# google/supersonic

Hardware: AMD Instinct MI355X
Metric: rows/sec filter->project->aggregate, 100M x 8 INT64/DOUBLE (higher is better)
Workload: dtype int64/f64; 1 GPU; Q-FPA-wide: SUM(a+b),COUNT(*),SUM(c),MIN(d),MAX(d0),SUM(d1),SUM(d2*d3) WHERE a>499 over a device-resident 100000000-row x 8-col block per GPU; rows_per_gpu=100000000, parallelism=single GPU, tile_rows=512, grid=768, lds_bytes=35568, specialized_stages=1

## Files before the change

supersonic_amd/csrc/launch.h:

```cpp
#ifndef SSGPU_LAUNCH_H_
#define SSGPU_LAUNCH_H_

#ifndef __HIPCC_RTC__
#include <hip/hip_runtime_api.h>
#include <stdint.h>
#endif
#include "vm.h"

enum SlotKind {
  SLOT_SUM_INT = 0, SLOT_SUM_DD = 1, SLOT_MIN_U64 = 2, SLOT_MAX_U64 = 3, SLOT_MIN_F64 = 4,
  SLOT_MAX_F64 = 5, SLOT_FIRST = 6, SLOT_LAST = 7, SLOT_COUNT = 8
};
enum EmitKind {
  EMIT_U64 = 0, EMIT_I64KEY = 1, EMIT_U32 = 2, EMIT_I32KEY = 3, EMIT_F64 = 4, EMIT_F32 = 5,
  EMIT_DD_F64 = 6, EMIT_DD_F32 = 7, EMIT_U8 = 8,
  EMIT_DDRES_F64 = 9,
  EMIT_CNT_U64 = 20, EMIT_CNT_U32 = 21,
  EMIT_FKEY_F64 = 100, EMIT_FKEY_F32 = 101
};
#define SSGPU_STATE_ARRAYS 8

struct EmitDesc { void* data; uint8_t* is_null; int slot; int out_kind; };

struct GroupKeyOut { void* data; uint8_t* is_null; uint32_t shift, bits, nullbit, width; };
// ... 165 lines not shown
                                    bool prefetch = false);
hipError_t ssgpu_launch_group_resident_rtc(void* handle, const PartAggParams& A, const PlainScatterParams& S, int grid, hipStream_t stream);
hipError_t ssgpu_launch_part_agg_rtc(void* handle, const PartAggParams& P, hipStream_t stream);
void* ssgpu_rtc_specialize_pscat(int device, const PlainScatterParams& S, const PscatGeom& g, std::string* why);
hipError_t ssgpu_launch_part_scatter_plain_rtc(void* handle, const PlainScatterParams& P, const PscatGeom& g, int grid, hipStream_t stream);
void* ssgpu_rtc_function(void* handle);
void ssgpu_rtc_release(void* handle);
void ssgpu_rtc_cached_only(bool on);
void ssgpu_rtc_mode(int mode);
int ssgpu_rtc_current_mode();
bool ssgpu_rtc_pending();
void ssgpu_rtc_trim(int keep);
void ssgpu_rtc_stats(long long* modules, long long* code_bytes, long long* compilations, long long* disk_hits);
#endif
hipError_t ssgpu_pipeline_set_max_lds(int bytes);
hipError_t ssgpu_launch_finish_slots(const VmAccRec* partials, int n_slots, int n_parts, const int* slot_kind,
                                     VmAccRec* out, uint64_t* state , hipStream_t stream,
                                     const EmitDesc* descs = nullptr, int n_out = 0 );
hipError_t ssgpu_launch_slots_to_state(const VmAccRec* recs, int n_slots, const int* slot_kind, uint64_t* state,
                                       hipStream_t stream);
hipError_t ssgpu_launch_fold_state(const uint64_t* images, int n_images, uint64_t* state, int n_slots, const int* slot_kind, hipStream_t stream);
hipError_t ssgpu_launch_fold_emit(const uint64_t* images, int n_images, uint64_t* state, int n_slots, const int* slot_kind, VmAccRec* recs,
                                  const EmitDesc* descs, int n_out, hipStream_t stream);
hipError_t ssgpu_launch_state_to_slots(const uint64_t* state, int n_slots, const int* slot_kind, VmAccRec* recs,
                                       hipStream_t stream);
hipError_t ssgpu_launch_emit_scalar(const VmAccRec* recs, const EmitDesc* descs, int n_out, hipStream_t stream);
hipError_t ssgpu_launch_scan_counts(const uint32_t* in, uint32_t* out, int n, uint64_t* total, hipStream_t stream);
hipError_t ssgpu_launch_group_count(const GroupExtractParams& P, uint32_t* tile_counts, hipStream_t stream);
hipError_t ssgpu_launch_group_extract_lb(const GroupExtractParams& P, unsigned long long* status, uint64_t epoch, unsigned int* ctrl, unsigned int* error_flag, hipStream_t stream);
hipError_t ssgpu_launch_group_extract(const GroupExtractParams& P, hipStream_t stream);
hipError_t ssgpu_launch_fill_u64(uint64_t* p, uint64_t v, size_t n, hipStream_t stream);
hipError_t ssgpu_launch_fill_pattern_u64(uint64_t* p, const uint64_t* pattern, uint32_t plen, size_t n,
                                         hipStream_t stream);
// ... 93 lines not shown
```

supersonic_amd/csrc/pipeline_kernels.hip:

```cpp
#ifndef __HIPCC_RTC__
#include <hip/hip_runtime.h>
#include <stdint.h>
#endif
#include "vm.h"
#include "launch.h"
#ifdef SSGPU_RTC_NINSTR
#include "rtc_prog.h"
#endif

typedef unsigned long long u64;
typedef long long i64;
typedef unsigned int u32;
typedef int i32;
typedef unsigned char u8;

#ifdef SSGPU_PC_PROFILE
#define PC_PROF(...) __VA_ARGS__
#else
#define PC_PROF(...)
#endif
struct LdsBase {
  __device__ __forceinline__ char* operator+(u32 off) const {
    return (char*)(__attribute__((address_space(3))) char*)off;
  }
// ... 753 lines not shown
      a = dd_add_d(a, u2d(state[3 * n_slots + s]));
      r.v0 = d2u(a.hi); r.v1 = d2u(a.lo);
    } break;
    case SLOT_MIN_U64: r.v0 = state[4 * n_slots + s] ^ 0x8000000000000000ull; break;
    case SLOT_MAX_U64: r.v0 = state[5 * n_slots + s] ^ 0x8000000000000000ull; break;
    case SLOT_MIN_F64: r.v0 = state[6 * n_slots + s]; break;
    case SLOT_MAX_F64: r.v0 = state[7 * n_slots + s]; break;
    case SLOT_FIRST: r.v0 = state[s]; r.v1 = state[4 * n_slots + s] ^ 0x8000000000000000ull; break;
    case SLOT_LAST: r.v0 = state[s]; r.v1 = state[5 * n_slots + s] ^ 0x8000000000000000ull; break;
    default: break;
  }
  return r;
}

__device__ __forceinline__ void emit_scalar_one(const EmitDesc d, const VmAccRec r);
__global__ __launch_bounds__(256) void ssgpu_finish_slots_kernel(const VmAccRec* __restrict__ partials, int n_slots,
                                                                 int n_parts, const int* __restrict__ slot_kind,
                                                                 VmAccRec* __restrict__ out, u64* __restrict__ state,
                                                                 const EmitDesc* __restrict__ descs, int n_out) {
  __shared__ VmAccRec tree[256];
  const int s = blockIdx.x, t = threadIdx.x;
  const int kind = slot_kind[s];
  VmAccRec acc; acc.v0 = 0; acc.v1 = 0; acc.cnt = 0; acc.pad = 0;
  if (kind == SLOT_SUM_DD) { acc.v0 = d2u(-0.0); acc.v1 = d2u(0.0); }
  for (int i = t; i < n_parts; i += 256) {
    const VmAccRec r = partials[((size_t)(i / VM_WAVES) * n_slots + s) * VM_WAVES + (i % VM_WAVES)];
    combine_rec(kind, acc, r);
  }
  tree[t] = acc;
  __syncthreads();
  for (int stride = 128; stride > 0; stride >>= 1) {
    if (t < stride) { VmAccRec a = tree[t]; combine_rec(kind, a, tree[t + stride]); tree[t] = a; }
    __syncthreads();
  }
  if (t == 0) { out[s] = tree[0]; if (state) slot_to_state(tree[0], kind, s, n_slots, state); }
  if (descs)
    for (int i = t; i < n_out; i += 256) { const EmitDesc d = descs[i]; if (d.slot == s) emit_scalar_one(d, tree[0]); }
}

__global__ void ssgpu_slots_to_state_kernel(const VmAccRec* __restrict__ recs, int n_slots,
                                            const int* __restrict__ slot_kind, u64* __restrict__ state) {
  int s = blockIdx.x * blockDim.x + threadIdx.x;
  if (s >= n_slots) return;
  slot_to_state(recs[s], slot_kind[s], s, n_slots, state);
}
__global__ void ssgpu_state_to_slots_kernel(const u64* __restrict__ state, int n_slots,
                                            const int* __restrict__ slot_kind, VmAccRec* __restrict__ recs) {
  int s = blockIdx.x * blockDim.x + threadIdx.x;
  if (s >= n_slots) return;
  recs[s] = state_to_slot(state, slot_kind[s], s, n_slots);
}

// ... 955 lines not shown
  e = hipFuncSetAttribute(reinterpret_cast<const void*>(ssgpu_part_agg_kernel<SSGPU_PART_MAX_WORDS>), hipFuncAttributeMaxDynamicSharedMemorySize, bytes);
  if (e != hipSuccess) return e;
  return hipFuncSetAttribute(reinterpret_cast<const void*>(ssgpu_part_agg_kernel<16>), hipFuncAttributeMaxDynamicSharedMemorySize, bytes);
}
hipError_t ssgpu_pipeline_set_max_lds(int bytes) {
  hipError_t e;
  e = hipFuncSetAttribute(reinterpret_cast<const void*>(ssgpu_pipeline_kernel<1, false>), hipFuncAttributeMaxDynamicSharedMemorySize, bytes); if (e != hipSuccess) return e;
  e = hipFuncSetAttribute(reinterpret_cast<const void*>(ssgpu_pipeline_kernel<2, false>), hipFuncAttributeMaxDynamicSharedMemorySize, bytes); if (e != hipSuccess) return e;
  e = hipFuncSetAttribute(reinterpret_cast<const void*>(ssgpu_pipeline_kernel<4, false>), hipFuncAttributeMaxDynamicSharedMemorySize, bytes); if (e != hipSuccess) return e;
  e = hipFuncSetAttribute(reinterpret_cast<const void*>(ssgpu_pipeline_kernel<1, true>), hipFuncAttributeMaxDynamicSharedMemorySize, bytes); if (e != hipSuccess) return e;
  e = hipFuncSetAttribute(reinterpret_cast<const void*>(ssgpu_pipeline_kernel<2, true>), hipFuncAttributeMaxDynamicSharedMemorySize, bytes); if (e != hipSuccess) return e;
  e = hipFuncSetAttribute(reinterpret_cast<const void*>(ssgpu_pipeline_kernel<4, true>), hipFuncAttributeMaxDynamicSharedMemorySize, bytes);
  return e;
}
hipError_t ssgpu_launch_finish_slots(const VmAccRec* partials, int n_slots, int n_parts, const int* slot_kind,
                                     VmAccRec* out, uint64_t* state, hipStream_t stream, const EmitDesc* descs, int n_out) {
  hipLaunchKernelGGL(ssgpu_finish_slots_kernel, dim3(n_slots), dim3(256), 0, stream, partials, n_slots, n_parts, slot_kind, out, (u64*)state, descs, n_out);
  return hipGetLastError();
}
hipError_t ssgpu_launch_slots_to_state(const VmAccRec* recs, int n_slots, const int* slot_kind, uint64_t* state, hipStream_t stream) {
  int blocks = (n_slots + 63) / 64;
  hipLaunchKernelGGL(ssgpu_slots_to_state_kernel, dim3(blocks), dim3(64), 0, stream, recs, n_slots, slot_kind, (u64*)state);
  return hipGetLastError();
}
__device__ __forceinline__ void fold_state_slot(const u64* __restrict__ images, int n_images, u64* __restrict__ state, int n_slots, int kind, int s);
__global__ __launch_bounds__(64) void ssgpu_fold_state_kernel(const u64* __restrict__ images, int n_images, u64* __restrict__ state,
                                                              int n_slots, const int* __restrict__ slot_kind) {
  const int s = blockIdx.x * 64 + threadIdx.x;
  if (s >= n_slots) return;
  fold_state_slot(images, n_images, state, n_slots, slot_kind[s], s);
}
__device__ __forceinline__ void fold_state_slot(const u64* __restrict__ images, int n_images, u64* __restrict__ state, int n_slots, int kind, int s) {
// ... 132 lines not shown
```

supersonic_amd/csrc/runtime.cpp:

```cpp
#include <hip/hip_runtime_api.h>

#include <atomic>
#include <chrono>
#include <map>
#include <tuple>
#include <set>
#include <mutex>
#include <stdio.h>
#include <string.h>
#include <algorithm>
#include <cmath>
#include <string>
#include <unistd.h>
#include <thread>
#include <unordered_set>
#include <vector>
#include <deque>
#include <functional>

#include "engine.h"

using namespace ssgpu;

#define HIP_TRY(ctx, expr)                                                          \
// ... 27 lines not shown
  int64_t part_wgs_per_cu = 0;
  int64_t part_lds_target = 0;
  int64_t sort_records = 1;
  int64_t sort_hybrid = 1;
  int64_t group_slab = 1;
  int64_t group_scout = 1;
  int64_t group_scout_rows = 8 << 20;
  int64_t group_resident = 1;
  int64_t group_dense = 1;
  int64_t dense_parts = 0;
  int64_t dense_min_rows = 1 << 16;
  int64_t async_handoff = 1;
  int64_t lazy_feedback = 0;
  int64_t part_prefetch = 1;
  int64_t fuse_emit = 1;
  int64_t pscat_pipe = 1;
  int64_t pscat_threads = 0, pscat_rows = 0, pscat_wgs = 0;
  int64_t part_plain = 1;
  int64_t sort_compact = 1;
  int64_t sort_hi_digits = 4;
  int64_t part_agg_lds = 0;
  int64_t profile = 1;
  int64_t profile_total = 1;
  int64_t debug_timing = 0;
  int64_t specialize = 3;
  int64_t specialize_min_rows = 1 << 22;
};

struct MemQuota { int64_t limit = -1; int64_t used = 0; };
static thread_local MemQuota* g_quota = nullptr;
// ... 79 lines not shown
      (void)hipGetLastError();
      int dev = -1;
      if (hipGetDevice(&dev) == hipSuccess && g_pool.trim(dev) > 0) e = hipMalloc(&p, want);
    }
    if (e == hipSuccess) { cap = want; q = Q; g_dev_bytes.fetch_add((long long)want); if (q) q->used += (int64_t)want; } else p = nullptr;
    return e;
  }
  template <typename T> T* as() const { return reinterpret_cast<T*>(p); }
};

struct PinnedBuf {
  void* p = nullptr;
  size_t cap = 0;
  ~PinnedBuf() { drop(); }
  void drop() { if (p) { (void)hipHostFree(p); g_pinned_bytes.fetch_sub((long long)cap); } p = nullptr; cap = 0; }
  hipError_t ensure(size_t bytes) {
    if (bytes <= cap && p) return hipSuccess;
    drop();
    size_t want = std::max<size_t>(bytes, 256);
    hipError_t e = hipHostMalloc(&p, want, hipHostMallocDefault);
    if (e == hipSuccess) { cap = want; g_pinned_bytes.fetch_add((long long)want); } else p = nullptr;
    return e;
  }
};

struct OutCol { DevBuf data, nulls; bool nullable = false; uint32_t width = 8; };

struct StageExec {
  DevBuf prog_main, prog_count;
  struct RtcSlot {
    void* h = nullptr; bool tried = false; uint32_t static_lds = 0, tag = 0;
    int missed_mode = -1;
    bool stronger_mode_now() const { if (h || missed_mode < 0) return false; const int m = ssgpu_rtc_current_mode(); return missed_mode == 1 && m != 1; }
    bool pending = false; std::chrono::steady_clock::time_point next_poll{};
    void drop() { if (h) ssgpu_rtc_release(h); h = nullptr; tried = false; static_lds = 0; tag = 0; pending = false; missed_mode = -1; }
// ... 48 lines not shown
    uint32_t span[8] = {0}, stride[8] = {0};
    uint64_t slots = 0;
    uint32_t np = 0, cap = 0;
    uint64_t chunk_bytes = 0;
    int64_t widened = 0;
  } dense;
  DevBuf dense_dom, dense_flags;
  void* dense_table = nullptr;
  std::vector<DevBuf> rowid_tmp;
  std::vector<DevBuf> jkeys, jkeys_hi, jrows, jmisc;
  std::vector<DevBuf> jcounts, jstarts, jslot_of_row, jrows_sorted;
  DevBuf jx_offsets, jx_lhs_idx, jx_rhs_row;
  std::vector<VmJoin> vm_joins;
  uint32_t capacity = 0;
  DevBuf error_flag;
  DevBuf debug, debug_pc, total2;
  DevBuf skeys_a, skeys_b, skeys_c, sidx_a, sidx_b, shist, soffs, seg_id, sstatus, sticket, srecs, dflag;
  DevBuf rank_first, rank_of_seg, rank_row, rank_own;
  DevBuf seg_counts, seg_offsets, seg_total;
  DevBuf route_scratch;
  uint64_t sort_epoch = 0;
  bool emit_ready = false;
  bool emitted_with_finish = false;
  bool pattern_ready = false;
  DevBuf out_arena;
  std::vector<OutCol> out;
  int64_t out_rows = -1;
  const void* out_rows_dev = nullptr;
  int64_t out_capacity = 0;
  int last_group_shape = 0;
// ... 74 lines not shown
        if (consumed[b]) (void)hipEventDestroy(consumed[b]);
        uploaded[b] = consumed[b] = nullptr; in_flight[b] = false;
      }
    }
  } host_stream;
  struct StreamJob {
    int kind = 0;
    ssgpu_plan* head = nullptr; ssgpu_plan* tail = nullptr;
    std::vector<DevBuf> acc_data, acc_nulls;
    int64_t acc_rows = 0, acc_cap = 0;
    int64_t rows_hint = 0;
  };
  StreamJob* stream_job = nullptr;
  ssgpu_plan* skip_plan = nullptr;
  int64_t run_row_end = 0;
  bool keep_error_flags = false;
  ssgpu_result result;
};

struct ssgpu_block {
  ssgpu_ctx* ctx = nullptr;
  Schema schema;
  int64_t capacity = 0, rows = 0;
  DevBuf arena;
  std::vector<DevBuf> data, nulls;
  ssgpu_dict* dict = nullptr;
};
static const size_t kBlockColumnSkew = 512, kBlockArenaMin = 32u << 20;

static int fail(ssgpu_ctx* ctx, const Status& s) { if (ctx) ctx->err = s.msg; return s.code; }
// ... 82 lines not shown
  else if (k == "part_lds_target") c->part_lds_target = value;
  else if (k == "part_agg_lds") c->part_agg_lds = value;
  else if (k == "group_slab") c->group_slab = value;
  else if (k == "group_resident") c->group_resident = value;
  else if (k == "group_dense") c->group_dense = value;
  else if (k == "dense_parts") c->dense_parts = value;
  else if (k == "dense_min_rows") c->dense_min_rows = value;
  else if (k == "group_scout") c->group_scout = value;
  else if (k == "group_scout_rows") c->group_scout_rows = value;
  else if (k == "part_plain") c->part_plain = value;
  else if (k == "pscat_threads") c->pscat_threads = value;
  else if (k == "pscat_rows") c->pscat_rows = value;
  else if (k == "pscat_wgs") c->pscat_wgs = value;
  else if (k == "pscat_pipe") c->pscat_pipe = value;
  else if (k == "fuse_emit") c->fuse_emit = value;
  else if (k == "part_prefetch") c->part_prefetch = value;
  else if (k == "lazy_feedback") c->lazy_feedback = value;
  else if (k == "async_handoff") c->async_handoff = value;
  else if (k == "sort_records") c->sort_records = value;
  else if (k == "sort_hybrid") c->sort_hybrid = value;
  else if (k == "sort_hi_digits") c->sort_hi_digits = value;
  else if (k == "sort_compact") c->sort_compact = value;
  else if (k == "group_capacity") {
    int64_t cap = 1; while (cap < value) cap <<= 1;
    c->group_capacity = cap;
  } else if (k == "profile") c->profile = value;
  else if (k == "profile_total") c->profile_total = value;
  else if (k == "debug_timing") c->debug_timing = value;
  else if (k == "specialize") c->specialize = value;
  else if (k == "specialize_min_rows") c->specialize_min_rows = value < 0 ? 0 : value;
// ... 453 lines not shown
}

void ssgpu_plan_destroy(ssgpu_plan* p) {
  if (!p) return;
  if (p->skip_plan) { ssgpu_plan* q = p->skip_plan; p->skip_plan = nullptr; ssgpu_plan_destroy(q); }
  if (p->stream_job) {
    ssgpu_plan::StreamJob* j = p->stream_job; p->stream_job = nullptr;
    if (p->ctx && p->ctx->device >= 0) (void)hipStreamSynchronize(p->ctx->stream);
    if (j->tail) ssgpu_plan_destroy(j->tail);
    if (j->head && j->head != p) ssgpu_plan_destroy(j->head);
    delete j;
  }
  if (p->ctx && p->ctx->device >= 0) {
    (void)hipStreamSynchronize(p->ctx->stream);
    if (p->host_stream.open) { (void)hipStreamSynchronize(p->ctx->copy_stream); p->host_stream.drop_events(); p->host_stream.open = false; }
    if (p->ev_begin) { (void)hipEventDestroy(p->ev_begin); g_events.fetch_sub(1); }
    if (p->ev_end) { (void)hipEventDestroy(p->ev_end); g_events.fetch_sub(1); }
    for (int i = 0; i < ssgpu_plan::kEventRing; ++i) {
      if (p->ring0[i]) { (void)hipEventDestroy(p->ring0[i]); g_events.fetch_sub(1); }
      if (p->ring1[i]) { (void)hipEventDestroy(p->ring1[i]); g_events.fetch_sub(1); }
    }
  }
  for (auto& ex : p->exec) { ex.rtc_main.drop(); ex.rtc_pscatter.drop(); ex.rtc_plain.drop(); ex.rtc_part.drop(); ex.rtc_resident.drop(); ex.rtc_hot.drop(); }
  for (auto& ex : p->exec) if (ex.fb_event) { (void)hipEventDestroy(ex.fb_event); ex.fb_event = nullptr; g_events.fetch_sub(1); }
  ssgpu_ctx* c = p->ctx;
  g_live_plans.fetch_sub(1);
  if (c && c->device >= 0) (void)hipSetDevice(c->device);
  tls_park_released = c && c->device >= 0;
  delete p;
  tls_park_released = false;
// ... 91 lines not shown
  ProgramLayout L = layout_program(st.main, c->opt);
  if (ex.prog_main.p && L.K == ex.lay.K) return SSGPU_OK;
  ex.lay = L;
  int rc = upload_program(c, st.main, L, &ex.prog_main, &ex.n_instr_main, &p->host_prog_scratch);
  if (rc != SSGPU_OK) return rc;
  ex.host_prog_main = p->host_prog_scratch;
  if (ex.rtc_main.h) (void)hipStreamSynchronize(c->stream);
  ex.rtc_main.drop(); ex.rtc_why.clear();
  if (!st.count_pass.empty()) {
    LowerOptions o = c->opt; o.tile_rows = VM_TILE_UNIT * 4;
    ex.lay_count = layout_program(st.count_pass, o);
    if (ex.lay_count.K < L.K) { o.tile_rows = VM_TILE_UNIT * L.K; ex.lay_count = layout_program(st.count_pass, o); }
    rc = upload_program(c, st.count_pass, ex.lay_count, &ex.prog_count, &ex.n_instr_count, &p->host_prog_scratch);
    if (rc != SSGPU_OK) return rc;
  }
  HIP_TRY(c, ex.error_flag.ensure(sizeof(uint32_t)));
  return SSGPU_OK;
}

int sort_rows_by_u32(ssgpu_plan* p, StageExec& ex, const uint32_t* keys32, uint64_t n, uint32_t** sorted) {
  ssgpu_ctx* c = p->ctx;
  const uint32_t nt = ssgpu_sort_tiles(n);
  HIP_TRY(c, ex.skeys_a.ensure(std::max<uint64_t>(n, 1) * 8)); HIP_TRY(c, ex.skeys_b.ensure(std::max<uint64_t>(n, 1) * 8));
  HIP_TRY(c, ex.sidx_a.ensure(std::max<uint64_t>(n, 1) * 4)); HIP_TRY(c, ex.sidx_b.ensure(std::max<uint64_t>(n, 1) * 4));
  HIP_TRY(c, ex.shist.ensure((size_t)std::max<uint32_t>(nt, 1) * 256 * 4)); HIP_TRY(c, ex.soffs.ensure((size_t)std::max<uint32_t>(nt, 1) * 256 * 4));
  HIP_TRY(c, ex.total.ensure(8)); HIP_TRY(c, ex.total2.ensure(16));
  uint64_t* ka = ex.skeys_a.as<uint64_t>(); uint64_t* kb = ex.skeys_b.as<uint64_t>();
  uint32_t* ia = ex.sidx_a.as<uint32_t>(); uint32_t* ib = ex.sidx_b.as<uint32_t>();
  HIP_TRY(c, ssgpu_launch_sort_iota(ia, n, c->stream));
  if (n > 0) {
    const unsigned long long init[2] = {0ull, ~0ull};
// ... 363 lines not shown
  }
  P.wg_partials = ex.wg_partials.as<VmAccRec>();
  P.error_flag = ex.error_flag.as<unsigned int>();
  if (c->debug_timing) {
    HIP_TRY(c, ex.debug.ensure((size_t)grid * 4 * 8));
    P.debug = ex.debug.as<unsigned long long>();
  }
  { int rc = attach_pc_profile(c, ex, &P); if (rc != SSGPU_OK) return rc; }
  if (c->profile) HIP_TRY(c, hipEventRecord(p->ev_dom0, c->stream));
  HIP_TRY(c, launch_main(p, st, ex, P, ex.lay.K, grid));
  if (c->profile) HIP_TRY(c, hipEventRecord(p->ev_dom1, c->stream));
  { int rc = print_pc_profile(c, ex, st.main, P.n_instr); if (rc != SSGPU_OK) return rc; }
  int n_emit = 0;
  ex.emitted_with_finish = false;
  if (!stop_at_partial && c->fuse_emit) { const int rc = prepare_scalar_emit(p, si, &n_emit); if (rc != SSGPU_OK) return rc; ex.emitted_with_finish = true; }
  HIP_TRY(c, ssgpu_launch_finish_slots(ex.wg_partials.as<VmAccRec>(), ns, grid * VM_WAVES, ex.slot_kind.as<int>(),
                                       ex.slot_recs.as<VmAccRec>(), stop_at_partial ? ex.state.as<uint64_t>() : nullptr, c->stream,
                                       ex.emitted_with_finish ? ex.emit_descs.as<EmitDesc>() : nullptr, n_emit));
  p->counters.n_launches += 2;
  p->counters.tile_rows = P.tile_rows; p->counters.grid = grid; p->counters.lds_bytes = (int32_t)ex.lay.lds_bytes;
  if (c->debug_timing) {
    std::vector<unsigned long long> dbg((size_t)grid * 4);
    HIP_TRY(c, hipMemcpy(dbg.data(), ex.debug.p, dbg.size() * 8, hipMemcpyDeviceToHost));
    double tot = 0, wait = 0, tiles = 0;
    for (int g = 0; g < grid; ++g) { tot += (double)dbg[g * 4]; wait += (double)dbg[g * 4 + 1]; tiles += (double)dbg[g * 4 + 2]; }
    fprintf(stderr, "[ssgpu debug] grid=%d tiles/wg=%.1f cycles/wg=%.0f wait=%.1f%% cycles/tile=%.0f (wait %.0f)\n", grid, tiles / grid,
            tot / grid, 100.0 * wait / tot, tot / tiles, wait / tiles);
  }
  return SSGPU_OK;
}

static const int64_t kSeqSumPiece = 1 << 21;
static int run_seq_sums(ssgpu_plan* p, Stage& st, StageExec& ex, const InCols& in, const uint32_t* seg_id) {
// ... 1312 lines not shown
static const void* rows_word(const StageExec& ex) { return ex.out_rows_dev ? ex.out_rows_dev : ex.total.p; }
int stage_rows(ssgpu_plan* p, size_t si, int64_t* rows) {
  ssgpu_ctx* c = p->ctx; StageExec& ex = p->exec[si];
  if (ex.out_rows < 0) {
    uint64_t total = 0;
    HIP_TRY(c, hipMemcpyAsync(&total, rows_word(ex), 8, hipMemcpyDeviceToHost, c->stream));
    HIP_TRY(c, hipStreamSynchronize(c->stream));
    ex.out_rows = (int64_t)total;
  }
  *rows = ex.out_rows;
  return SSGPU_OK;
}

int check_error_flags(ssgpu_plan* p);

int check_error_flags(ssgpu_plan* p) {
  ssgpu_ctx* c = p->ctx;
  std::vector<uint32_t> flags(p->exec.size(), 0);
  for (size_t i = 0; i < p->exec.size(); ++i)
    if (p->exec[i].error_flag.p)
      HIP_TRY(c, hipMemcpyAsync(&flags[i], p->exec[i].error_flag.p, 4, hipMemcpyDeviceToHost, c->stream));
  HIP_TRY(c, hipStreamSynchronize(c->stream));
  for (uint32_t& f : flags) {
    if (f & SSGPU_FLAG_NAN_IN_MINMAX) p->nan_seen = true;
    f &= 0xFFu;
  }
  for (uint32_t f : flags) {
    if (f == 3) { c->err = "decoupled look-back: a tile waited for an earlier tile's row count for too long and gave up"; return SSGPU_ERROR_HIP; }
    if (f) {
      c->err = f == 2 ? "Evaluation error: invalid argument of a signaling math expression (negative input of SQRT)"
                      : "Evaluation error: division by zero in a signaling expression";
      return SSGPU_ERROR_EVALUATION_ERROR;
    }
  }
  return SSGPU_OK;
}

// ... 39 lines not shown
  p->exec.clear();
  p->stages = stages; p->describe = describe;
  p->exec.resize(p->stages.size());
  std::vector<ssgpu_column> cols = p->last_cols;
  int rc = run_plan(p, cols.data(), (int32_t)cols.size(), p->last_rows, p->last_base, false);
  if (rc != SSGPU_OK) return rc;
  rc = settle_plan(p);
  if (rc != SSGPU_OK) return rc;
  rc = check_error_flags(p);
  p->nan_seen = false;
  return rc;
}

int run_plan(ssgpu_plan* p, const ssgpu_column* cols, int32_t n_cols, int64_t rows, int64_t row_id_base, bool partial) {
  ssgpu_ctx* c = p->ctx;
  if (!c || c->device < 0) { if (c) c->err = "no gfx950 device bound to this context (bind-only context)"; return SSGPU_ERROR_NO_DEVICE; }
  ssgpu_rtc_mode(!p->cached_only ? 0 : p->background && rows >= p->background_min_rows ? 2 : 1);
  p->run_row_end = row_id_base + rows;
  p->nan_seen = false;
  if (p->deferred) {
    p->deferred = false;
    for (auto& ex : p->exec) {
      if (!ex.fb_pending) continue;
      if (ex.fb_event) HIP_TRY(c, hipEventSynchronize(ex.fb_event)); else HIP_TRY(c, hipStreamSynchronize(c->stream));
      const uint32_t* fb = static_cast<const uint32_t*>(ex.fb_host.p);
      const int kind = ex.fb_pending; ex.fb_pending = 0;
      if (fb[0] || (kind == 2 && (fb[1] || fb[3]))) ex.steady = 0;
      else if (kind == 1 && (uint64_t)fb[1] > 2ull * ex.steady_bypass + (uint64_t)(p->last_rows >> 6)) ex.steady = 0;
    }
  }
// ... 13 lines not shown
    c->err = "partial runs need a plan whose only stage is a ScalarAggregate"; return SSGPU_ERROR_NOT_IMPLEMENTED;
  }
  for (size_t si = 0; si < p->stages.size(); ++si) {
    if (si == 0) ++p->n_runs;
    int rc = prepare_stage(p, si);
    if (rc != SSGPU_OK) return rc;
  }
  if (c->profile) {
    const int slot = (int)(p->profiled_runs % ssgpu_plan::kEventRing);
    if (!p->ring0[slot]) { HIP_TRY(c, hipEventCreate(&p->ring0[slot])); HIP_TRY(c, hipEventCreate(&p->ring1[slot])); g_events.fetch_add(2); }
    p->ev_dom0 = p->ring0[slot]; p->ev_dom1 = p->ring1[slot];
    ++p->profiled_runs;
    p->events_valid = false;
    if (c->profile_total) HIP_TRY(c, hipEventRecord(p->ev_begin, c->stream));
  }
  for (size_t si = 0; si < p->exec.size(); ++si)
    if (p->exec[si].error_flag.p && !p->keep_error_flags && !(si == 0 && p->stages[si].kind == STAGE_GROUP_AGG)) HIP_TRY(c, hipMemsetAsync(p->exec[si].error_flag.p, 0, sizeof(uint32_t), c->stream));
  int64_t alg_bytes = 0;
  for (size_t si = 0; si < p->stages.size(); ++si) {
    if (p->interrupted.exchange(0)) { c->err = "interrupted"; return SSGPU_INTERRUPTED; }
    Stage& st = p->stages[si];
    int rc = SSGPU_OK;
    alg_bytes += st.algorithmic_bytes_per_row * in.rows;
    rc = build_joins(p, st, p->exec[si]);
    if (rc != SSGPU_OK) return rc;
    switch (st.kind) {
      case STAGE_SCALAR_AGG:
        rc = run_scalar_agg(p, si, in, row_id_base, partial);
        if (rc == SSGPU_OK && !partial) rc = emit_scalar_agg(p, si);
        if (rc == SSGPU_OK && !partial && !st.seq_sums.empty()) rc = run_seq_sums(p, st, p->exec[si], in, nullptr);
        break;
      case STAGE_MATERIALIZE: rc = run_materialize(p, si, in, row_id_base); break;
// ... 29 lines not shown
  }
  if (c->profile && c->profile_total) { HIP_TRY(c, hipEventRecord(p->ev_end, c->stream)); p->events_valid = true; }
  p->counters.algorithmic_bytes = alg_bytes;
  p->last_rows = rows;
  p->last_cols.assign(cols, cols + n_cols); p->last_base = row_id_base; p->last_partial = partial;
  p->partial_pending = partial;
  return SSGPU_OK;
}

}

extern "C" {

int ssgpu_plan_run(ssgpu_plan* p, const ssgpu_column* cols, int32_t n_cols, int64_t rows, ssgpu_result** out) {
  if (!p) return SSGPU_ERROR_INVALID_ARGUMENT_VALUE;
  int rc = run_plan(p, cols, n_cols, rows, 0, false);
  if (rc != SSGPU_OK) return rc;
  if (!p->lazy_feedback) {
    rc = settle_plan(p);
    if (rc != SSGPU_OK) return rc;
    (void)check_error_flags(p);
    rc = fix_nan_minmax(p);
    if (rc != SSGPU_OK) return rc;
  }
  if (out) *out = &p->result;
  return SSGPU_OK;
}

int ssgpu_plan_run_best_effort(ssgpu_plan* p, const ssgpu_column* cols, int32_t n_cols, int64_t rows, int64_t start_row, int64_t* next_row, ssgpu_result** out) {
  if (!p || !next_row) return SSGPU_ERROR_INVALID_ARGUMENT_VALUE;
// ... 747 lines not shown
  p->last_cols.clear(); p->last_rows = rows;
  return settle_plan(p) == SSGPU_OK ? check_error_flags(p) : SSGPU_ERROR_HIP;
}

int ssgpu_plan_set_aux_input(ssgpu_plan* p, const ssgpu_column* cols, int32_t n_cols, int64_t rows) {
  if (!p) return SSGPU_ERROR_INVALID_ARGUMENT_VALUE;
  if (n_cols != (int)p->desc.aux_schema.size()) { p->ctx->err = "column count does not match the plan's auxiliary schema"; return SSGPU_ERROR_ATTRIBUTE_COUNT_MISMATCH; }
  if (rows < 0 || rows >= (int64_t)VM_NONE) { p->ctx->err = "auxiliary input: bad row count"; return SSGPU_ERROR_INVALID_ARGUMENT_VALUE; }
  p->aux_cols.assign(cols, cols + n_cols);
  p->aux_rows = rows;
  return SSGPU_OK;
}

int ssgpu_plan_run_partial(ssgpu_plan* p, const ssgpu_column* cols, int32_t n_cols, int64_t rows, int64_t base) {
  if (!p) return SSGPU_ERROR_INVALID_ARGUMENT_VALUE;
  return run_plan(p, cols, n_cols, rows, base, true);
}

static int dense_stage_of(ssgpu_plan* p, bool need_device) {
  if (!p) return SSGPU_ERROR_INVALID_ARGUMENT_VALUE;
  ssgpu_ctx* c = p->ctx;
  if (need_device && (!c || c->device < 0)) { if (c) c->err = "no gfx950 device bound to this context (bind-only context)"; return SSGPU_ERROR_NO_DEVICE; }
  if (p->stages.size() != 1 || p->stages[0].kind != STAGE_GROUP_AGG || !dense_eligible(c, p->stages[0])) {
    c->err = "dense slots need a plan that is ONE plain GroupAggregate stage over integer-like key columns"; return SSGPU_ERROR_NOT_IMPLEMENTED;
  }
  for (auto& a : p->stages[0].aggs) if (a.gather_col >= 0) { c->err = "FIRST / LAST aggregates take their values from the shard that saw the row: not in the dense exchange"; return SSGPU_ERROR_NOT_IMPLEMENTED; }
  return SSGPU_OK;
}
int ssgpu_plan_key_ranges(ssgpu_plan* p, const ssgpu_column* cols, int32_t n_cols, int64_t rows, int32_t* n_keys, uint64_t* lo, uint64_t* hi) {
  int rc = dense_stage_of(p, true);
// ... 593 lines not shown
    offsets[4 * n] = -1; offsets[4 * n + 1] = -1; offsets[4 * n + 2] = L.valid_off; offsets[4 * n + 3] = -1;
  }
  return SSGPU_OK;
}

int ssgpu_result_pack_image(ssgpu_result* r, int64_t capacity_rows, void* image) {
  if (!r || !r->plan || r->plan->exec.empty() || !image) return SSGPU_ERROR_INVALID_ARGUMENT_VALUE;
  ssgpu_plan* p = r->plan; ssgpu_ctx* c = p->ctx;
  if (c->device < 0) return SSGPU_ERROR_NO_DEVICE;
  ImageLayout L;
  if (!image_layout(p->result_schema, capacity_rows, 1, &L)) { c->err = "result images need fixed-width columns and a non-negative capacity"; return SSGPU_ERROR_INVALID_ARGUMENT_VALUE; }
  StageExec& ex = p->exec.back();
  ImagePackParams P; memset(&P, 0, sizeof(P));
  P.image = image; P.capacity = (unsigned long long)capacity_rows;
  if (ex.out_rows >= 0) P.rows_host = (unsigned long long)ex.out_rows; else P.rows_dev = static_cast<const unsigned long long*>(rows_word(ex));
  for (auto& sx : p->exec) if (sx.error_flag.p && P.n_flags < 8) P.error_flags[P.n_flags++] = sx.error_flag.as<unsigned int>();
  for (auto& sx : p->exec) if (sx.fb_pending && sx.goverflow.p && P.n_retry + 2 <= 4) {
    P.retry_flags[P.n_retry++] = sx.goverflow.as<unsigned int>();
    if (sx.fb_pending == 2) P.retry_flags[P.n_retry++] = sx.goverflow.as<unsigned int>() + 1;
  }
  for (size_t i = 0; i < ex.out.size(); ++i) {
    ImagePiece& d = P.pieces[P.n_pieces++];
    d.src = ex.out[i].data.p; d.image_off = (unsigned long long)L.img_data[i]; d.width = L.width[i];
    if (L.img_null[i] >= 0) {
      ImagePiece& z = P.pieces[P.n_pieces++];
      z.src = ex.out[i].nullable ? ex.out[i].nulls.p : nullptr; z.image_off = (unsigned long long)L.img_null[i]; z.width = 1;
    }
  }
  HIP_TRY(c, ssgpu_launch_pack_image(P, c->stream));
  return SSGPU_OK;
}

int ssgpu_result_route_images(ssgpu_result* r, int32_t n_keys, int32_t n_dest, int64_t capacity_rows, void* images) {
  if (!r || !r->plan || r->plan->exec.empty() || !images || n_dest < 1 || n_dest > 256 || n_keys < 0 || n_keys > 16) return SSGPU_ERROR_INVALID_ARGUMENT_VALUE;
  ssgpu_plan* p = r->plan; ssgpu_ctx* c = p->ctx;
  if (c->device < 0) return SSGPU_ERROR_NO_DEVICE;
  if (n_keys > (int32_t)p->result_schema.size()) return SSGPU_ERROR_INVALID_ARGUMENT_VALUE;
  ImageLayout L;
  if (!image_layout(p->result_schema, capacity_rows, 1, &L)) { c->err = "result images need fixed-width columns and a non-negative capacity"; return SSGPU_ERROR_INVALID_ARGUMENT_VALUE; }
  StageExec& ex = p->exec.back();
  ImagePackParams P; memset(&P, 0, sizeof(P));
  ImageRoutePieces R; memset(&R, 0, sizeof(R));
  P.image = images; P.capacity = (unsigned long long)capacity_rows;
  const uint64_t rows_max = ex.out_rows >= 0 ? (uint64_t)ex.out_rows : (uint64_t)std::max<int64_t>(ex.out_capacity, 1);
  P.rows_host = rows_max;
  if (ex.out_rows < 0) P.rows_dev = static_cast<const unsigned long long*>(rows_word(ex));
  for (auto& sx : p->exec) if (sx.error_flag.p && P.n_flags < 8) P.error_flags[P.n_flags++] = sx.error_flag.as<unsigned int>();
  for (auto& sx : p->exec) if (sx.fb_pending && sx.goverflow.p && P.n_retry + 2 <= 4) {
    P.retry_flags[P.n_retry++] = sx.goverflow.as<unsigned int>();
    if (sx.fb_pending == 2) P.retry_flags[P.n_retry++] = sx.goverflow.as<unsigned int>() + 1;
  }
  for (size_t i = 0; i < ex.out.size(); ++i) {
    if ((int32_t)i < n_keys) { R.key_piece[i] = P.n_pieces; R.key_null_piece[i] = -1; }
    ImagePiece& d = P.pieces[P.n_pieces++];
    d.src = ex.out[i].data.p; d.image_off = (unsigned long long)L.img_data[i]; d.width = L.width[i];
    if (L.img_null[i] >= 0) {
      if ((int32_t)i < n_keys) R.key_null_piece[i] = (int)P.n_pieces;
      ImagePiece& z = P.pieces[P.n_pieces++];
      z.src = ex.out[i].nullable ? ex.out[i].nulls.p : nullptr; z.image_off = (unsigned long long)L.img_null[i]; z.width = 1;
    }
  }
  R.n_keys = (unsigned)n_keys; R.n_dest = (unsigned)n_dest; R.image_bytes = (unsigned long long)L.image_bytes;
// ... 38 lines not shown
```

Measured before the change: 104.0 billion rows/s.

## Latch error flags in finish kernel and publish to coherent host word

The finish-slots kernel now atomically swaps the error flag to zero, copies it into a second word, and publishes it with an epoch to a coherent pinned host word. For single-stage scalar aggregates, this lets the host skip the per-run memset and the device-to-host flag copy. The finish kernel also batches its partial loads 16 per thread and replaces the shared-memory tree tail with wave shuffles. This adds epoch-tracking state and a fallback path, and a stale epoch forces the old memcpy route.

```diff
diff --git a/supersonic_amd/csrc/launch.h b/supersonic_amd/csrc/launch.h
--- a/supersonic_amd/csrc/launch.h
+++ b/supersonic_amd/csrc/launch.h
@@ -203,9 +203,11 @@
 void ssgpu_rtc_stats(long long* modules, long long* code_bytes, long long* compilations, long long* disk_hits);
 #endif
 hipError_t ssgpu_pipeline_set_max_lds(int bytes);
+struct FinishLatch { unsigned int* words = nullptr; uint64_t* host_word = nullptr; unsigned int epoch = 0; };
 hipError_t ssgpu_launch_finish_slots(const VmAccRec* partials, int n_slots, int n_parts, const int* slot_kind,
                                      VmAccRec* out, uint64_t* state , hipStream_t stream,
-                                     const EmitDesc* descs = nullptr, int n_out = 0 );
+                                     const EmitDesc* descs = nullptr, int n_out = 0 ,
+                                     const FinishLatch& latch = FinishLatch(), int form = 1 );
 hipError_t ssgpu_launch_slots_to_state(const VmAccRec* recs, int n_slots, const int* slot_kind, uint64_t* state,
                                        hipStream_t stream);
 hipError_t ssgpu_launch_fold_state(const uint64_t* images, int n_images, uint64_t* state, int n_slots, const int* slot_kind, hipStream_t stream);
diff --git a/supersonic_amd/csrc/pipeline_kernels.hip b/supersonic_amd/csrc/pipeline_kernels.hip
--- a/supersonic_amd/csrc/pipeline_kernels.hip
+++ b/supersonic_amd/csrc/pipeline_kernels.hip
@@ -791,10 +791,10 @@
 }
 
 __device__ __forceinline__ void emit_scalar_one(const EmitDesc d, const VmAccRec r);
-__global__ __launch_bounds__(256) void ssgpu_finish_slots_kernel(const VmAccRec* __restrict__ partials, int n_slots,
-                                                                 int n_parts, const int* __restrict__ slot_kind,
-                                                                 VmAccRec* __restrict__ out, u64* __restrict__ state,
-                                                                 const EmitDesc* __restrict__ descs, int n_out) {
+__global__ __launch_bounds__(256) void ssgpu_finish_slots_ref_kernel(const VmAccRec* __restrict__ partials, int n_slots,
+                                                                     int n_parts, const int* __restrict__ slot_kind,
+                                                                     VmAccRec* __restrict__ out, u64* __restrict__ state,
+                                                                     const EmitDesc* __restrict__ descs, int n_out) {
   __shared__ VmAccRec tree[256];
   const int s = blockIdx.x, t = threadIdx.x;
   const int kind = slot_kind[s];
@@ -813,6 +813,63 @@
   if (t == 0) { out[s] = tree[0]; if (state) slot_to_state(tree[0], kind, s, n_slots, state); }
   if (descs)
     for (int i = t; i < n_out; i += 256) { const EmitDesc d = descs[i]; if (d.slot == s) emit_scalar_one(d, tree[0]); }
+}
+
+static constexpr int FINISH_BATCH = 16;
+__global__ __launch_bounds__(256) void ssgpu_finish_slots_kernel(const VmAccRec* __restrict__ partials, int n_slots,
+                                                                 int n_parts, const int* __restrict__ slot_kind,
+                                                                 VmAccRec* __restrict__ out, u64* __restrict__ state,
+                                                                 const EmitDesc* __restrict__ descs, int n_out,
+                                                                 unsigned int* latch, u64* host_word, unsigned int epoch) {
+  __shared__ VmAccRec tree[128];
+  const int s = blockIdx.x, t = threadIdx.x;
+  const int kind = slot_kind[s];
+  EmitDesc d0; d0.data = nullptr; d0.is_null = nullptr; d0.slot = -1; d0.out_kind = 0;
+  if (descs && t < n_out) d0 = descs[t];
+  const bool latcher = latch && s == 0 && t == 0;
+  unsigned int latched = 0;
+  if (latcher) latched = atomicExch(latch, 0u);
+  VmAccRec acc; acc.v0 = 0; acc.v1 = 0; acc.cnt = 0; acc.pad = 0;
+  if (kind == SLOT_SUM_DD) { acc.v0 = d2u(-0.0); acc.v1 = d2u(0.0); }
+  for (int base = t; base < n_parts; base += 256 * FINISH_BATCH) {
+    ulonglong2 a[FINISH_BATCH], b[FINISH_BATCH];
+#pragma unroll
+    for (int k = 0; k < FINISH_BATCH; ++k) {
+      const int i = base + k * 256;
+      a[k] = make_ulonglong2(0, 0); b[k] = make_ulonglong2(0, 0);
+      if (i < n_parts) {
+        const ulonglong2* q = reinterpret_cast<const ulonglong2*>(partials + (((size_t)(i / VM_WAVES) * n_slots + s) * VM_WAVES + (i % VM_WAVES)));
+        a[k] = q[0]; b[k] = q[1];
+      }
+    }
+#pragma unroll
+    for (int k = 0; k < FINISH_BATCH; ++k) {
+      if (base + k * 256 < n_parts) { VmAccRec r; r.v0 = a[k].x; r.v1 = a[k].y; r.cnt = b[k].x; r.pad = b[k].y; combine_rec(kind, acc, r); }
+    }
+  }
+  if (t >= 128) tree[t - 128] = acc;
+  __syncthreads();
+  if (t < 128) { combine_rec(kind, acc, tree[t]); if (t >= 64) tree[t] = acc; }
+  __syncthreads();
+  if (t < 64) {
+    combine_rec(kind, acc, tree[t + 64]);
+#pragma unroll
+    for (int stride = 32; stride > 0; stride >>= 1) {
+      VmAccRec r; r.v0 = __shfl_down(acc.v0, stride); r.v1 = __shfl_down(acc.v1, stride); r.cnt = __shfl_down(acc.cnt, stride); r.pad = 0;
+      if (t < stride) combine_rec(kind, acc, r);
+    }
+  }
+  if (t == 0) { out[s] = acc; if (state) slot_to_state(acc, kind, s, n_slots, state); tree[0] = acc; }
+  if (descs) {
+    __syncthreads();
+    const VmAccRec fin = tree[0];
+    if (d0.slot == s) emit_scalar_one(d0, fin);
+    for (int i = t + 256; i < n_out; i += 256) { const EmitDesc d = descs[i]; if (d.slot == s) emit_scalar_one(d, fin); }
+  }
+  if (latcher) {
+    latch[1] = latched;
+    if (host_word) __hip_atomic_store(host_word, ((u64)epoch << 32) | (u64)latched, __ATOMIC_RELEASE, __HIP_MEMORY_SCOPE_SYSTEM);
+  }
 }
 
 __global__ void ssgpu_slots_to_state_kernel(const VmAccRec* __restrict__ recs, int n_slots,
@@ -1798,8 +1855,15 @@
   return e;
 }
 hipError_t ssgpu_launch_finish_slots(const VmAccRec* partials, int n_slots, int n_parts, const int* slot_kind,
-                                     VmAccRec* out, uint64_t* state, hipStream_t stream, const EmitDesc* descs, int n_out) {
-  hipLaunchKernelGGL(ssgpu_finish_slots_kernel, dim3(n_slots), dim3(256), 0, stream, partials, n_slots, n_parts, slot_kind, out, (u64*)state, descs, n_out);
+                                     VmAccRec* out, uint64_t* state, hipStream_t stream, const EmitDesc* descs, int n_out,
+                                     const FinishLatch& latch, int form) {
+  if (form == 0 && !latch.words)
+    hipLaunchKernelGGL(ssgpu_finish_slots_ref_kernel, dim3(n_slots), dim3(256), 0, stream, partials, n_slots, n_parts, slot_kind, out, (u64*)state, descs, n_out);
+  else if (form == 0)
+    return hipErrorInvalidValue;
+  else
+    hipLaunchKernelGGL(ssgpu_finish_slots_kernel, dim3(n_slots), dim3(256), 0, stream, partials, n_slots, n_parts, slot_kind, out, (u64*)state, descs, n_out,
+                       latch.words, (u64*)latch.host_word, latch.epoch);
   return hipGetLastError();
 }
 hipError_t ssgpu_launch_slots_to_state(const VmAccRec* recs, int n_slots, const int* slot_kind, uint64_t* state, hipStream_t stream) {
diff --git a/supersonic_amd/csrc/runtime.cpp b/supersonic_amd/csrc/runtime.cpp
--- a/supersonic_amd/csrc/runtime.cpp
+++ b/supersonic_amd/csrc/runtime.cpp
@@ -65,6 +65,7 @@
   int64_t lazy_feedback = 0;
   int64_t part_prefetch = 1;
   int64_t fuse_emit = 1;
+  int64_t finish_form = 1;
   int64_t pscat_pipe = 1;
   int64_t pscat_threads = 0, pscat_rows = 0, pscat_wgs = 0;
   int64_t part_plain = 1;
@@ -174,11 +175,11 @@
   size_t cap = 0;
   ~PinnedBuf() { drop(); }
   void drop() { if (p) { (void)hipHostFree(p); g_pinned_bytes.fetch_sub((long long)cap); } p = nullptr; cap = 0; }
-  hipError_t ensure(size_t bytes) {
+  hipError_t ensure(size_t bytes, unsigned int flags = hipHostMallocDefault) {
     if (bytes <= cap && p) return hipSuccess;
     drop();
     size_t want = std::max<size_t>(bytes, 256);
-    hipError_t e = hipHostMalloc(&p, want, hipHostMallocDefault);
+    hipError_t e = hipHostMalloc(&p, want, flags);
     if (e == hipSuccess) { cap = want; g_pinned_bytes.fetch_add((long long)want); } else p = nullptr;
     return e;
   }
@@ -257,6 +258,8 @@
   std::vector<VmJoin> vm_joins;
   uint32_t capacity = 0;
   DevBuf error_flag;
+  bool flag_latched = false;
+  bool flag_raw_clean = false;
   DevBuf debug, debug_pc, total2;
   DevBuf skeys_a, skeys_b, skeys_c, sidx_a, sidx_b, shist, soffs, seg_id, sstatus, sticket, srecs, dflag;
   DevBuf rank_first, rank_of_seg, rank_row, rank_own;
@@ -361,6 +364,9 @@
   StreamJob* stream_job = nullptr;
   ssgpu_plan* skip_plan = nullptr;
   int64_t run_row_end = 0;
+  bool latch_next = false;
+  PinnedBuf latch_host;
+  uint32_t latch_epoch = 0;
   bool keep_error_flags = false;
   ssgpu_result result;
 };
@@ -473,6 +479,7 @@
   else if (k == "pscat_wgs") c->pscat_wgs = value;
   else if (k == "pscat_pipe") c->pscat_pipe = value;
   else if (k == "fuse_emit") c->fuse_emit = value;
+  else if (k == "finish_form") c->finish_form = value;
   else if (k == "part_prefetch") c->part_prefetch = value;
   else if (k == "lazy_feedback") c->lazy_feedback = value;
   else if (k == "async_handoff") c->async_handoff = value;
@@ -956,6 +963,7 @@
   if (p->ctx && p->ctx->device >= 0) {
     (void)hipStreamSynchronize(p->ctx->stream);
     if (p->host_stream.open) { (void)hipStreamSynchronize(p->ctx->copy_stream); p->host_stream.drop_events(); p->host_stream.open = false; }
+    p->latch_host.drop();
     if (p->ev_begin) { (void)hipEventDestroy(p->ev_begin); g_events.fetch_sub(1); }
     if (p->ev_end) { (void)hipEventDestroy(p->ev_end); g_events.fetch_sub(1); }
     for (int i = 0; i < ssgpu_plan::kEventRing; ++i) {
@@ -1077,7 +1085,7 @@
     rc = upload_program(c, st.count_pass, ex.lay_count, &ex.prog_count, &ex.n_instr_count, &p->host_prog_scratch);
     if (rc != SSGPU_OK) return rc;
   }
-  HIP_TRY(c, ex.error_flag.ensure(sizeof(uint32_t)));
+  HIP_TRY(c, ex.error_flag.ensure(2 * sizeof(uint32_t)));
   return SSGPU_OK;
 }
 
@@ -1471,9 +1479,12 @@
   int n_emit = 0;
   ex.emitted_with_finish = false;
   if (!stop_at_partial && c->fuse_emit) { const int rc = prepare_scalar_emit(p, si, &n_emit); if (rc != SSGPU_OK) return rc; ex.emitted_with_finish = true; }
+  FinishLatch latch;
+  if (ex.flag_latched) { latch.words = ex.error_flag.as<unsigned int>(); latch.host_word = static_cast<uint64_t*>(p->latch_host.p); latch.epoch = p->latch_epoch; }
   HIP_TRY(c, ssgpu_launch_finish_slots(ex.wg_partials.as<VmAccRec>(), ns, grid * VM_WAVES, ex.slot_kind.as<int>(),
                                        ex.slot_recs.as<VmAccRec>(), stop_at_partial ? ex.state.as<uint64_t>() : nullptr, c->stream,
-                                       ex.emitted_with_finish ? ex.emit_descs.as<EmitDesc>() : nullptr, n_emit));
+                                       ex.emitted_with_finish ? ex.emit_descs.as<EmitDesc>() : nullptr, n_emit, latch, c->finish_form != 0 ? 1 : 0));
+  if (ex.flag_latched) ex.flag_raw_clean = true;
   p->counters.n_launches += 2;
   p->counters.tile_rows = P.tile_rows; p->counters.grid = grid; p->counters.lds_bytes = (int32_t)ex.lay.lds_bytes;
   if (c->debug_timing) {
@@ -2816,13 +2827,27 @@
 
 int check_error_flags(ssgpu_plan* p);
 
+static unsigned int* flag_word(StageExec& ex) { return ex.error_flag.as<unsigned int>() + (ex.flag_latched ? 1 : 0); }
+
+static bool plan_latched(const ssgpu_plan* p) { return p->exec.size() == 1 && p->exec[0].flag_latched && p->latch_host.p; }
+static bool latched_flags(const ssgpu_plan* p, uint32_t* flags) {
+  const uint64_t w = __atomic_load_n(static_cast<const uint64_t*>(p->latch_host.p), __ATOMIC_ACQUIRE);
+  if ((uint32_t)(w >> 32) != p->latch_epoch) return false;
+  *flags = (uint32_t)w;
+  return true;
+}
+
 int check_error_flags(ssgpu_plan* p) {
   ssgpu_ctx* c = p->ctx;
   std::vector<uint32_t> flags(p->exec.size(), 0);
-  for (size_t i = 0; i < p->exec.size(); ++i)
-    if (p->exec[i].error_flag.p)
-      HIP_TRY(c, hipMemcpyAsync(&flags[i], p->exec[i].error_flag.p, 4, hipMemcpyDeviceToHost, c->stream));
-  HIP_TRY(c, hipStreamSynchronize(c->stream));
+  const bool latched = plan_latched(p);
+  if (latched) HIP_TRY(c, hipStreamSynchronize(c->stream));
+  if (!latched || !latched_flags(p, &flags[0])) {
+    for (size_t i = 0; i < p->exec.size(); ++i)
+      if (p->exec[i].error_flag.p)
+        HIP_TRY(c, hipMemcpyAsync(&flags[i], flag_word(p->exec[i]), 4, hipMemcpyDeviceToHost, c->stream));
+    HIP_TRY(c, hipStreamSynchronize(c->stream));
+  }
   for (uint32_t& f : flags) {
     if (f & SSGPU_FLAG_NAN_IN_MINMAX) p->nan_seen = true;
     f &= 0xFFu;
@@ -2892,6 +2917,7 @@
 
 int run_plan(ssgpu_plan* p, const ssgpu_column* cols, int32_t n_cols, int64_t rows, int64_t row_id_base, bool partial) {
   ssgpu_ctx* c = p->ctx;
+  const bool latch_req = p->latch_next; p->latch_next = false;
   if (!c || c->device < 0) { if (c) c->err = "no gfx950 device bound to this context (bind-only context)"; return SSGPU_ERROR_NO_DEVICE; }
   ssgpu_rtc_mode(!p->cached_only ? 0 : p->background && rows >= p->background_min_rows ? 2 : 1);
   p->run_row_end = row_id_base + rows;
@@ -2935,8 +2961,20 @@
     p->events_valid = false;
     if (c->profile_total) HIP_TRY(c, hipEventRecord(p->ev_begin, c->stream));
   }
-  for (size_t si = 0; si < p->exec.size(); ++si)
+  const bool latch = latch_req && c->finish_form != 0 && p->stages.size() == 1 && p->stages[0].kind == STAGE_SCALAR_AGG && !p->keep_error_flags &&
+                     p->stages[0].seq_sums.empty() && p->stages[0].distinct_cols.empty() && p->stages[0].main.n_slots > 0 && p->exec[0].error_flag.p;
+  if (latch) {
+    StageExec& ex = p->exec[0];
+    if (!p->latch_host.p) { HIP_TRY(c, p->latch_host.ensure(sizeof(uint64_t), hipHostMallocCoherent)); *static_cast<uint64_t*>(p->latch_host.p) = 0; }
+    if (!ex.flag_raw_clean) HIP_TRY(c, hipMemsetAsync(ex.error_flag.p, 0, 2 * sizeof(uint32_t), c->stream));
+    ex.flag_raw_clean = false;
+    ex.flag_latched = true;
+    p->latch_epoch = (uint32_t)p->n_runs;
+  }
+  for (size_t si = 0; si < p->exec.size() && !latch; ++si) {
+    p->exec[si].flag_latched = false; p->exec[si].flag_raw_clean = false;
     if (p->exec[si].error_flag.p && !p->keep_error_flags && !(si == 0 && p->stages[si].kind == STAGE_GROUP_AGG)) HIP_TRY(c, hipMemsetAsync(p->exec[si].error_flag.p, 0, sizeof(uint32_t), c->stream));
+  }
   int64_t alg_bytes = 0;
   for (size_t si = 0; si < p->stages.size(); ++si) {
     if (p->interrupted.exchange(0)) { c->err = "interrupted"; return SSGPU_INTERRUPTED; }
@@ -2996,6 +3034,7 @@
 
 int ssgpu_plan_run(ssgpu_plan* p, const ssgpu_column* cols, int32_t n_cols, int64_t rows, ssgpu_result** out) {
   if (!p) return SSGPU_ERROR_INVALID_ARGUMENT_VALUE;
+  p->latch_next = true;
   int rc = run_plan(p, cols, n_cols, rows, 0, false);
   if (rc != SSGPU_OK) return rc;
   if (!p->lazy_feedback) {
@@ -3773,6 +3812,7 @@
 
 int ssgpu_plan_run_partial(ssgpu_plan* p, const ssgpu_column* cols, int32_t n_cols, int64_t rows, int64_t base) {
   if (!p) return SSGPU_ERROR_INVALID_ARGUMENT_VALUE;
+  p->latch_next = true;
   return run_plan(p, cols, n_cols, rows, base, true);
 }
 
@@ -4396,7 +4436,7 @@
   ImagePackParams P; memset(&P, 0, sizeof(P));
   P.image = image; P.capacity = (unsigned long long)capacity_rows;
   if (ex.out_rows >= 0) P.rows_host = (unsigned long long)ex.out_rows; else P.rows_dev = static_cast<const unsigned long long*>(rows_word(ex));
-  for (auto& sx : p->exec) if (sx.error_flag.p && P.n_flags < 8) P.error_flags[P.n_flags++] = sx.error_flag.as<unsigned int>();
+  for (auto& sx : p->exec) if (sx.error_flag.p && P.n_flags < 8) P.error_flags[P.n_flags++] = flag_word(sx);
   for (auto& sx : p->exec) if (sx.fb_pending && sx.goverflow.p && P.n_retry + 2 <= 4) {
     P.retry_flags[P.n_retry++] = sx.goverflow.as<unsigned int>();
     if (sx.fb_pending == 2) P.retry_flags[P.n_retry++] = sx.goverflow.as<unsigned int>() + 1;
@@ -4427,7 +4467,7 @@
   const uint64_t rows_max = ex.out_rows >= 0 ? (uint64_t)ex.out_rows : (uint64_t)std::max<int64_t>(ex.out_capacity, 1);
   P.rows_host = rows_max;
   if (ex.out_rows < 0) P.rows_dev = static_cast<const unsigned long long*>(rows_word(ex));
-  for (auto& sx : p->exec) if (sx.error_flag.p && P.n_flags < 8) P.error_flags[P.n_flags++] = sx.error_flag.as<unsigned int>();
+  for (auto& sx : p->exec) if (sx.error_flag.p && P.n_flags < 8) P.error_flags[P.n_flags++] = flag_word(sx);
   for (auto& sx : p->exec) if (sx.fb_pending && sx.goverflow.p && P.n_retry + 2 <= 4) {
     P.retry_flags[P.n_retry++] = sx.goverflow.as<unsigned int>();
     if (sx.fb_pending == 2) P.retry_flags[P.n_retry++] = sx.goverflow.as<unsigned int>() + 1;
```

Result: no change. 104.3 billion rows/s, median of 6 (+0.3%).
